# snap-research/InstantRestore

Measured on AMD Instinct MI355X. Metric: restored images/sec @512px, 4 refs, single-step; 1/2/4/8 MI355X, higher is better.
Workload: dtype bf16

## Files before the change

### instantrestore_amd/csrc/linear_tiled.hip

```cpp
#include <stdlib.h>
#include <type_traits>

#include "ir_common.h"
#include "ir_colstats.h"
#include "ir_kernels.h"

namespace {

constexpr int kTiledPitch = 144;

template <typename T, int WM, int WN, int MI, int NI, bool XF32, bool ILV, int KW = 1>
__global__ void __launch_bounds__(WM * WN * KW * 64, KW == 1 ? 2 : 1) linear_tiled_kernel(const LinearKParams p) {
  using Tr = ElemTraits<T>;
  using v8 = typename Tr::v8;
  using v4 = typename Tr::v4;
  constexpr int NW = WM * WN, NT = NW * 64;
  constexpr int BM = WM * MI * 32, BN = WN * NI * 32;
  constexpr int XT = BM * 128, WT = BN * 128, STAGE = XT + WT;
  constexpr int XP = BM / 8 / NW, WP = BN / 8 / NW;
  constexpr int XU = BM * 8 / NT;
  static_assert(BM % (8 * NW) == 0 && BN % (8 * NW) == 0, "pieces must divide over the waves");
  extern __shared__ __attribute__((aligned(16))) unsigned char dsm_tiled[];
  const int lane = threadIdx.x & 63;
  const int wid_all = __builtin_amdgcn_readfirstlane(threadIdx.x >> 6);
  const int kg = KW == 1 ? 0 : wid_all / NW;
  const int wid = KW == 1 ? wid_all : wid_all - kg * NW;
  const int tid = wid * 64 + lane;
  unsigned char* const smem = dsm_tiled + kg * (2 * STAGE);

  const int wm = wid / WN, wn = wid - wm * WN;
  const int hi = lane >> 5, lq = lane & 31;

  const int MT = (p.M + BM - 1) / BM, NTl = p.N / BN;
  const int logical = xcd_remap((int)blockIdx.x, MT * NTl);
  const int GM = p.nsplit;
  const int grp = logical / (GM * NTl), rem = logical - grp * (GM * NTl);
  const int gm = (MT - grp * GM) < GM ? (MT - grp * GM) : GM;
  const int tm = grp * GM + rem % gm, tn = rem / gm;
  const int m0 = tm * BM, n0 = tn * BN;
  const int rows_valid = (p.M - m0) < BM ? (p.M - m0) : BM;
  const int KT = (p.K >> 6) / KW;
  const int kt0 = kg * KT;

  const T* const wbase = (const T*)p.w + (int64_t)n0 * p.w_ld;
  const i32x4 wrs = make_rsrc_words(wbase, (unsigned)(((int64_t)(BN - 1) * p.w_ld + p.K) * 2));
  unsigned wvo[WP];
#pragma unroll
  for (int j = 0; j < WP; ++j) {
    const int row = 8 * (wid + j * NW) + (lane >> 3);
    wvo[j] = (unsigned)(row * p.w_ld * 2 + ((((lane & 7) ^ ((row >> 1) & 7))) << 4));
  }
  i32x4 xrs = wrs;
  unsigned xvo[XF32 ? 1 : XP];
  const float* xfp[XF32 ? XU : 1];
  int xlds[XF32 ? XU : 1];
  if constexpr (!XF32) {
    const T* const xbase = (const T*)p.x + (int64_t)m0 * p.x_ld;
    xrs = make_rsrc_words(xbase, (unsigned)(((int64_t)(rows_valid - 1) * p.x_ld + p.K) * 2));
#pragma unroll
    for (int j = 0; j < XP; ++j) {
      const int row = 8 * (wid + j * NW) + (lane >> 3);
      xvo[j] = (unsigned)(row * p.x_ld * 2 + ((((lane & 7) ^ ((row >> 1) & 7))) << 4));
    }
  } else {
#pragma unroll
    for (int j = 0; j < XU; ++j) {
      const int u = tid + j * NT, row = u >> 3, ch = u & 7;
      const int gr = (m0 + row) < p.M ? (m0 + row) : (p.M - 1);
      xfp[j] = (const float*)p.x + (int64_t)gr * p.x_ld + ch * 8;
      xlds[j] = row * 128 + ((ch ^ ((row >> 1) & 7)) << 4);
    }
  }
  constexpr int NPIECE = WP + (XF32 ? 0 : XP);
  auto issue_piece = [&](int j, int kt, int slot) {
    unsigned char* const sx = smem + slot * STAGE;
    if (j < WP) buffer_load_lds16_async(wrs, sx + XT + (wid + j * NW) * 1024, wvo[j] + (kt0 + kt) * 128);
    else if constexpr (!XF32) buffer_load_lds16_async(xrs, sx + (wid + (j - WP) * NW) * 1024, xvo[j - WP] + (kt0 + kt) * 128);
  };
  auto issue_dma = [&](int kt, int slot) {
#pragma unroll
    for (int j = 0; j < NPIECE; ++j) issue_piece(j, kt, slot);
  };
  f32x4 xr[XF32 ? XU : 1][2];
  auto load_x32 = [&](int kt) {
    if constexpr (XF32) {
#pragma unroll
      for (int j = 0; j < XU; ++j) {
        asm volatile("global_load_dwordx4 %0, %1, off" : "=v"(xr[j][0]) : "v"(xfp[j] + (kt0 + kt) * 64) : "memory");
        asm volatile("global_load_dwordx4 %0, %1, off offset:16" : "=v"(xr[j][1]) : "v"(xfp[j] + (kt0 + kt) * 64) : "memory");
      }
    }
  };
  auto put_x32 = [&](int slot) {
    if constexpr (XF32) {
      unsigned char* const sx = smem + slot * STAGE;
      asm volatile("s_waitcnt vmcnt(0)" : "+v"(xr[0][0]), "+v"(xr[0][1]) : : "memory");
#pragma unroll
      for (int j = 1; j < XU; ++j) asm volatile("" : "+v"(xr[j][0]), "+v"(xr[j][1]));
#pragma unroll
      for (int j = 0; j < XU; ++j) {
        const f32x8 f = __builtin_shufflevector(xr[j][0], xr[j][1], 0, 1, 2, 3, 4, 5, 6, 7);
        *(IR_LDS v8*)(IR_LDS unsigned char*)(sx + xlds[j]) = __builtin_convertvector(f, v8);
      }
    }
  };

  int fread[4];
#pragma unroll
  for (int ks = 0; ks < 4; ++ks) fread[ks] = lq * 128 + (((2 * ks + hi) ^ ((lq >> 1) & 7)) << 4);
  const int xrow0 = wm * (MI * 32) * 128, wrow0 = XT + wn * (NI * 32) * 128;

  f32x16 acc[MI][NI];
#pragma unroll
  for (int mi = 0; mi < MI; ++mi)
#pragma unroll
    for (int ni = 0; ni < NI; ++ni)
#pragma unroll
      for (int r = 0; r < 16; ++r) acc[mi][ni][r] = 0.f;

  constexpr int HALF_MFMA = 2 * MI * NI;
  constexpr int STRIDE = (HALF_MFMA / NPIECE) > 0 ? (HALF_MFMA / NPIECE) : 1;
  auto compute = [&](int slot, int dma_kt, int dma_slot) {
    const unsigned char* const st = smem + slot * STAGE;
    v8 wf[2][NI], xf[2][MI];
    auto rd = [&](int ks, int b) {
#pragma unroll
      for (int ni = 0; ni < NI; ++ni) wf[b][ni] = *(const IR_LDS v8*)(IR_LDS unsigned char*)(st + wrow0 + ni * 4096 + fread[ks]);
#pragma unroll
      for (int mi = 0; mi < MI; ++mi) xf[b][mi] = *(const IR_LDS v8*)(IR_LDS unsigned char*)(st + xrow0 + mi * 4096 + fread[ks]);
    };
    rd(0, 0);
#pragma unroll
    for (int ks = 0; ks < 4; ++ks) {
      if (ks + 1 < 4) rd(ks + 1, (ks + 1) & 1);
#pragma unroll
      for (int mi = 0; mi < MI; ++mi)
#pragma unroll
        for (int ni = 0; ni < NI; ++ni) {
          acc[mi][ni] = Tr::mfma(wf[ks & 1][ni], xf[ks & 1][mi], acc[mi][ni]);
          if constexpr (ILV) {
            const int m = ks * MI * NI + mi * NI + ni;
            if (m < HALF_MFMA && (m % STRIDE) == STRIDE - 1 && (m / STRIDE) < NPIECE) {
              __builtin_amdgcn_sched_barrier(0);
              if (dma_kt >= 0) issue_piece(m / STRIDE, dma_kt, dma_slot);
              __builtin_amdgcn_sched_barrier(0);
            }
            if (m == HALF_MFMA - 1) {
#pragma unroll
              for (int j = HALF_MFMA / STRIDE; j < NPIECE; ++j)
                if (dma_kt >= 0) issue_piece(j, dma_kt, dma_slot);
            }
          }
        }
    }
  };

  issue_dma(0, 0);
  load_x32(0);
  put_x32(0);
  asm volatile("s_waitcnt vmcnt(0)" ::: "memory");
  __syncthreads();
  for (int kt = 0; kt + 1 < KT; ++kt) {
    const int cur = kt & 1;
    if constexpr (!ILV) issue_dma(kt + 1, cur ^ 1);
    load_x32(kt + 1);
    compute(cur, kt + 1, cur ^ 1);
    put_x32(cur ^ 1);
    asm volatile("s_waitcnt vmcnt(0)" ::: "memory");
    __syncthreads();
  }
  compute((KT - 1) & 1, -1, 0);
  __syncthreads();
  if constexpr (KW == 2) {
    constexpr int HAND_OFF = 2 * STAGE;
    static_assert(2 * STAGE >= NW * MI * 32 * kTiledPitch, "epilogue staging must stay below the hand-over area");
    static_assert(2 * STAGE >= NW * MI * NI * 16 * 64 * 4, "hand-over area");
    unsigned char* const hand = dsm_tiled + HAND_OFF + wid * (MI * NI * 16 * 64 * 4) + lane * 16;
    if (kg == 1) {
#pragma unroll
      for (int mi = 0; mi < MI; ++mi)
#pragma unroll
        for (int ni = 0; ni < NI; ++ni)
#pragma unroll
          for (int g = 0; g < 4; ++g)
            *(f32x4_alias*)(hand + ((mi * NI + ni) * 4 + g) * 1024) = f32x4{acc[mi][ni][4 * g], acc[mi][ni][4 * g + 1], acc[mi][ni][4 * g + 2], acc[mi][ni][4 * g + 3]};
    }
    __syncthreads();
    if (kg == 1) return;
#pragma unroll
    for (int mi = 0; mi < MI; ++mi)
#pragma unroll
      for (int ni = 0; ni < NI; ++ni)
#pragma unroll
        for (int g = 0; g < 4; ++g) {
          const f32x4 o = *(const f32x4_alias*)(hand + ((mi * NI + ni) * 4 + g) * 1024);
#pragma unroll
          for (int i = 0; i < 4; ++i) acc[mi][ni][4 * g + i] += o[i];
        }
  }

  unsigned char* const tb = smem + wid * (MI * 32 * kTiledPitch);
  const int row_base = m0 + wm * (MI * 32);
  v4 bvs[NI][4];
  if (p.bias != nullptr) {
#pragma unroll
    for (int ni = 0; ni < NI; ++ni)
#pragma unroll
      for (int g = 0; g < 4; ++g) bvs[ni][g] = *(const v4*)((const T*)p.bias + n0 + wn * (NI * 32) + ni * 32 + 8 * g + 4 * hi);
  } else {
#pragma unroll
    for (int ni = 0; ni < NI; ++ni)
#pragma unroll
      for (int g = 0; g < 4; ++g) bvs[ni][g] = v4{0, 0, 0, 0};
  }
#pragma unroll
  for (int nh = 0; nh < NI / 2; ++nh) {
    const int ncol0 = n0 + wn * (NI * 32) + nh * 64;
#pragma unroll
    for (int n2 = 0; n2 < 2; ++n2) {
      const int ni = 2 * nh + n2;
      const float cs = (ncol0 + n2 * 32) < p.scale_cols ? p.col_scale : 1.0f;
#pragma unroll
      for (int g = 0; g < 4; ++g) {
        f32x4 bz;
#pragma unroll
        for (int i = 0; i < 4; ++i) bz[i] = (float)bvs[ni][g][i];
#pragma unroll
        for (int mi = 0; mi < MI; ++mi) {
          f32x4 f;
#pragma unroll
          for (int i = 0; i < 4; ++i) f[i] = acc[mi][ni][4 * g + i] * cs + bz[i];
          *(v4*)(tb + (mi * 32 + lq) * kTiledPitch + n2 * 64 + (8 * g + 4 * hi) * 2) = __builtin_convertvector(f, v4);
        }
      }
    }
    ir_wave_lds_fence();
    const int st_head = (ncol0 - p.st_col0) >> 6;
    const bool st_on = p.st_ws != nullptr && ncol0 >= p.st_col0 && st_head < (p.st_cols >> 6) && row_base < p.M;
    ColStatsAcc sacc;
#pragma unroll
    for (int j = 0; j < MI * 4; ++j) {
      const int r = 8 * j + (lane >> 3);
      const u32x4 v = *(const u32x4_alias*)(tb + r * kTiledPitch + (lane & 7) * 16);
      const int row = row_base + r;
      if (row < p.M) ir_store_y((u32x4*)((T*)p.y + (int64_t)row * p.y_ld + ncol0 + (lane & 7) * 8), v);
      if (st_on) {
        if (j == 0) ir_stats_first<T>(sacc, v);
        else ir_stats_add<T>(sacc, v);
      }
    }
    ir_wave_lds_fence();
    if (st_on) ir_stats_finish(sacc, p.st_ws + ((int64_t)(row_base / kStatsRows) * (p.st_cols >> 6) + st_head) * 128);
  }
}


template <typename T, bool XF32>
__global__ void __launch_bounds__(512, 2) linear_tiled_pp_kernel(const LinearKParams p) {
  using Tr = ElemTraits<T>;
  using v8 = typename Tr::v8;
  using v4 = typename Tr::v4;
  constexpr int NW = 8, NT = 512, WN = 2, MI = 2, NI = 4;
  constexpr int BM = 256, BN = 256;
  constexpr int XT = BM * 128, WT = BN * 128, STAGE = XT + WT;
  constexpr int XP = BM / 8 / NW, WP = BN / 8 / NW;
  constexpr int XU = BM * 8 / NT;
  constexpr int OUT_OFF = 2 * STAGE;
  extern __shared__ __attribute__((aligned(16))) unsigned char dsm_tiled_pp[];
  unsigned char* const smem = dsm_tiled_pp;

  const int tid = threadIdx.x;
  const int lane = tid & 63;
  const int wid = __builtin_amdgcn_readfirstlane(tid >> 6);
  const int grp = wid >> 2;
  const int wm = wid / WN, wn = wid - wm * WN;
  const int hi = lane >> 5, lq = lane & 31;
  const int KT = p.K >> 6;

  const int MT = (p.M + BM - 1) / BM, NTl = (p.N + BN - 1) / BN;
  const int ntiles = MT * NTl;
  const int xcd = blockIdx.x & 7, xs = blockIdx.x >> 3;
  const int q8 = ntiles >> 3, r8 = ntiles & 7;
  const int t_start = (xcd < r8) ? xcd * (q8 + 1) : r8 * (q8 + 1) + (xcd - r8) * q8;
  const int t_count = q8 + (xcd < r8 ? 1 : 0);
  const int wg_x = ((int)gridDim.x >> 3) + (xcd < ((int)gridDim.x & 7) ? 1 : 0);

  unsigned wvo[WP], xvo[XF32 ? 1 : XP];
  int xlds0 = 0;
#pragma unroll
  for (int j = 0; j < WP; ++j) {
    const int row = 8 * (wid + j * NW) + (lane >> 3);
    wvo[j] = (unsigned)(row * p.w_ld * 2 + ((((lane & 7) ^ ((row >> 1) & 7))) << 4));
  }
  if constexpr (!XF32) {
#pragma unroll
    for (int j = 0; j < XP; ++j) {
      const int row = 8 * (wid + j * NW) + (lane >> 3);
      xvo[j] = (unsigned)(row * p.x_ld * 2 + ((((lane & 7) ^ ((row >> 1) & 7))) << 4));
    }
  } else {
    const int row = tid >> 3, ch = tid & 7;
    xlds0 = row * 128 + ((ch ^ ((row >> 1) & 7)) << 4);
  }
  int fread[4];
#pragma unroll
  for (int ks = 0; ks < 4; ++ks) fread[ks] = lq * 128 + (((2 * ks + hi) ^ ((lq >> 1) & 7)) << 4);
  const int xrow0 = wm * (MI * 32) * 128, wrow0 = XT + wn * (NI * 32) * 128;

  int m0 = 0, n0 = 0;
  i32x4 wrs = {0, 0, 0, 0}, xrs = {0, 0, 0, 0};
  const float* xtile = nullptr;
  unsigned xoff[XF32 ? XU : 1];
  auto set_tile = [&](int logical) {
    const int GM = p.nsplit;
    const int tgrp = logical / (GM * NTl), rem = logical - tgrp * (GM * NTl);
    const int gm = (MT - tgrp * GM) < GM ? (MT - tgrp * GM) : GM;
    const int tm = tgrp * GM + rem % gm, tn = rem / gm;
    m0 = tm * BM; n0 = tn * BN;
    const int rows_valid = (p.M - m0) < BM ? (p.M - m0) : BM;
    const int cols_valid = (p.N - n0) < BN ? (p.N - n0) : BN;
    wrs = make_rsrc_words((const T*)p.w + (int64_t)n0 * p.w_ld, (unsigned)(((int64_t)(cols_valid - 1) * p.w_ld + p.K) * 2));
    if constexpr (!XF32) {
      xrs = make_rsrc_words((const T*)p.x + (int64_t)m0 * p.x_ld, (unsigned)(((int64_t)(rows_valid - 1) * p.x_ld + p.K) * 2));
    } else {
      xtile = (const float*)p.x + (int64_t)m0 * p.x_ld;
#pragma unroll
      for (int j = 0; j < XU; ++j) {
        const int row = (tid >> 3) + 64 * j;
        const int rr = row < rows_valid ? row : rows_valid - 1;
        xoff[j] = (unsigned)(rr * (int)p.x_ld + (tid & 7) * 8) * 4u;
      }
    }
  };
  f32x4 xr[XF32 ? XU : 1][2];
  auto issue_w = [&](int kt, int slot) {
    unsigned char* const sx = smem + slot * STAGE;
#pragma unroll
    for (int j = 0; j < WP; ++j) buffer_load_lds16_async(wrs, sx + XT + (wid + j * NW) * 1024, wvo[j] + kt * 128);
  };
  auto issue_x = [&](int kt, int slot) {
    if constexpr (!XF32) {
      unsigned char* const sx = smem + slot * STAGE;
#pragma unroll
      for (int j = 0; j < XP; ++j) buffer_load_lds16_async(xrs, sx + (wid + j * NW) * 1024, xvo[j] + kt * 128);
    } else {
#pragma unroll
      for (int j = 0; j < XU; ++j) {
        const unsigned o = xoff[j] + (unsigned)kt * 256u;
        asm volatile("s_nop 4\n\tglobal_load_dwordx4 %0, %1, %2" : "=v"(xr[j][0]) : "v"(o), "s"(xtile) : "memory");
        asm volatile("global_load_dwordx4 %0, %1, %2 offset:16" : "=v"(xr[j][1]) : "v"(o), "s"(xtile) : "memory");
      }
    }
  };
  auto land_stage = [&](int slot) {
    if constexpr (XF32) {
      unsigned char* const sx = smem + slot * STAGE;
      asm volatile("s_waitcnt vmcnt(0)" : "+v"(xr[0][0]), "+v"(xr[0][1]) : : "memory");
#pragma unroll
      for (int j = 1; j < XU; ++j) asm volatile("" : "+v"(xr[j][0]), "+v"(xr[j][1]));
#pragma unroll
      for (int j = 0; j < XU; ++j) {
        const f32x8 f = __builtin_shufflevector(xr[j][0], xr[j][1], 0, 1, 2, 3, 4, 5, 6, 7);
        *(IR_LDS v8*)(IR_LDS unsigned char*)(sx + xlds0 + j * 8192) = __builtin_convertvector(f, v8);
      }
    } else {
      asm volatile("s_waitcnt vmcnt(0)" ::: "memory");
    }
  };

  f32x16 acc[MI][NI];
  v8 wf[2][NI], xf[2][MI];
  auto load_frags = [&](int slot, int half) {
    const unsigned char* const st = smem + slot * STAGE;
#pragma unroll
    for (int q = 0; q < 2; ++q) {
#pragma unroll
      for (int ni = 0; ni < NI; ++ni) wf[q][ni] = *(const IR_LDS v8*)(IR_LDS unsigned char*)(st + wrow0 + ni * 4096 + fread[2 * half + q]);
#pragma unroll
      for (int mi = 0; mi < MI; ++mi) xf[q][mi] = *(const IR_LDS v8*)(IR_LDS unsigned char*)(st + xrow0 + mi * 4096 + fread[2 * half + q]);
    }
  };
  auto matrix_phase = [&]() {
    __builtin_amdgcn_s_setprio(1);
#pragma unroll
    for (int q = 0; q < 2; ++q)
#pragma unroll
      for (int mi = 0; mi < MI; ++mi)
#pragma unroll
        for (int ni = 0; ni < NI; ++ni) acc[mi][ni] = Tr::mfma(wf[q][ni], xf[q][mi], acc[mi][ni]);
    __builtin_amdgcn_s_setprio(0);
  };
  auto phase_end = [&]() {
    __builtin_amdgcn_sched_barrier(0);
    asm volatile("s_waitcnt lgkmcnt(0)" ::: "memory");
    __builtin_amdgcn_s_barrier();
    __builtin_amdgcn_sched_barrier(0);
  };
  auto epilogue = [&](int em0, int en0) {
    unsigned char* const tb = smem + OUT_OFF + wid * 4096;
#pragma unroll
    for (int nh = 0; nh < NI / 2; ++nh) {
      const int ncol0 = en0 + wn * (NI * 32) + nh * 64;
      if (ncol0 >= p.N) break;
      v4 bvs[2][4];
      if (p.bias != nullptr) {
#pragma unroll
        for (int n2 = 0; n2 < 2; ++n2)
#pragma unroll
          for (int g = 0; g < 4; ++g) bvs[n2][g] = *(const v4*)((const T*)p.bias + ncol0 + n2 * 32 + 8 * g + 4 * hi);
      } else {
#pragma unroll
        for (int n2 = 0; n2 < 2; ++n2)
#pragma unroll
          for (int g = 0; g < 4; ++g) bvs[n2][g] = v4{0, 0, 0, 0};
      }
      const int st_head = (ncol0 - p.st_col0) >> 6;
      const bool st_on = p.st_ws != nullptr && ncol0 >= p.st_col0 && st_head < (p.st_cols >> 6) && (em0 + wm * (MI * 32)) < p.M;
      ColStatsAcc sacc;
#pragma unroll
      for (int mi = 0; mi < MI; ++mi) {
#pragma unroll
        for (int half = 0; half < 2; ++half) {
          if ((lq >> 4) == half) {
#pragma unroll
            for (int n2 = 0; n2 < 2; ++n2) {
              const float cs = (ncol0 + n2 * 32) < p.scale_cols ? p.col_scale : 1.0f;
#pragma unroll
              for (int g = 0; g < 4; ++g) {
                f32x4 f;
#pragma unroll
                for (int i = 0; i < 4; ++i) f[i] = acc[mi][2 * nh + n2][4 * g + i] * cs + (float)bvs[n2][g][i];
                *(v4*)(tb + (lq & 15) * kTiledPitch + n2 * 64 + (8 * g + 4 * hi) * 2) = __builtin_convertvector(f, v4);
              }
            }
          }
          ir_wave_lds_fence();
#pragma unroll
          for (int j = 0; j < 2; ++j) {
            const int r = 8 * j + (lane >> 3);
            const u32x4 v = *(const u32x4_alias*)(tb + r * kTiledPitch + (lane & 7) * 16);
            const int row = em0 + wm * (MI * 32) + mi * 32 + half * 16 + r;
            if (row < p.M) ir_store_y((u32x4*)((T*)p.y + (int64_t)row * p.y_ld + ncol0 + (lane & 7) * 8), v);
            if (st_on) {
              if (mi == 0 && half == 0 && j == 0) ir_stats_first<T>(sacc, v);
              else ir_stats_add<T>(sacc, v);
            }
          }
          ir_wave_lds_fence();
        }
      }
      if (st_on) ir_stats_finish(sacc, p.st_ws + ((int64_t)((em0 + wm * (MI * 32)) / kStatsRows) * (p.st_cols >> 6) + st_head) * 128);
    }
  };

  if (xs >= t_count) return;
  set_tile(t_start + xs);
  issue_w(0, 0);
  issue_x(0, 0);
  for (int tl = xs; tl < t_count; tl += wg_x) {
#pragma unroll
    for (int mi = 0; mi < MI; ++mi)
#pragma unroll
      for (int ni = 0; ni < NI; ++ni)
#pragma unroll
        for (int r = 0; r < 16; ++r) acc[mi][ni][r] = 0.f;
    land_stage(0);
    asm volatile("s_waitcnt vmcnt(0)" ::: "memory");
    phase_end();
    load_frags(0, 0);
    if (KT > 1) { issue_w(1, 1); issue_x(1, 1); }
    if (grp == 1) phase_end();
    for (int kt = 0; kt < KT; ++kt) {
      const int cur = kt & 1;
      matrix_phase();
      phase_end();
      load_frags(cur, 1);
      if (kt + 1 < KT) land_stage(cur ^ 1);
      phase_end();
      matrix_phase();
      phase_end();
      if (kt + 1 < KT) {
        load_frags(cur ^ 1, 0);
        if (kt + 2 < KT) { issue_w(kt + 2, cur); issue_x(kt + 2, cur); }
      }
      phase_end();
    }
    if (grp == 0) phase_end();
    const int em0 = m0, en0 = n0;
    const bool more = tl + wg_x < t_count;
    if (more) {
      set_tile(t_start + tl + wg_x);
      issue_w(0, 0);
      if constexpr (!XF32) issue_x(0, 0);
    }
    epilogue(em0, en0);
    if constexpr (XF32) { if (more) issue_x(0, 0); }
  }
}


static int walk_group_rows() {
  static const int gm = [] { const char* e = getenv("IR_LIN_GM"); const int v = e ? atoi(e) : 0; return (v >= 1 && v <= 64) ? v : 4; }();
  return gm;
}

template <typename T, bool XF32>
hipError_t launch_pp(const LinearKParams& p0, hipStream_t s) {
  LinearKParams p = p0;
  p.nsplit = walk_group_rows();
  constexpr size_t dyn = 2 * (size_t)(256 + 256) * 128 + 8 * 4096;
  static IrOncePerDevice once;
  static std::atomic<int> n_cu[64];
  int dev = -1;
  const hipError_t ea = ir_opt_in_dynamic_lds(once, (const void*)linear_tiled_pp_kernel<T, XF32>, dyn, &dev);
  if (ea != hipSuccess) return ea;
  int cus = (dev >= 0 && dev < 64) ? n_cu[dev].load(std::memory_order_relaxed) : 0;
  if (cus <= 0) {
    if (hipDeviceGetAttribute(&cus, hipDeviceAttributeMultiprocessorCount, dev < 0 ? 0 : dev) != hipSuccess || cus <= 0) cus = 256;
    if (dev >= 0 && dev < 64) n_cu[dev].store(cus, std::memory_order_relaxed);
  }
  const int MT = (p.M + 255) / 256, NTl = (p.N + 255) / 256;
  const int ntiles = MT * NTl;
  static const bool persistent = [] { const char* e = getenv("IR_LIN_PERSISTENT"); return e == nullptr || e[0] != '0'; }();
  const int grid = (persistent && ntiles > cus) ? cus : ntiles;
  hipLaunchKernelGGL((linear_tiled_pp_kernel<T, XF32>), dim3((unsigned)grid), dim3(512), dyn, s, p);
  return hipGetLastError();
}

template <typename T, int WM, int WN, int MI, int NI, bool XF32, bool ILV, int KW = 1>
hipError_t launch_cfg(const LinearKParams& p0, hipStream_t s) {
  LinearKParams p = p0;
  p.nsplit = walk_group_rows();
  constexpr int BM = WM * MI * 32, BN = WN * NI * 32;
  constexpr size_t stage = (size_t)(BM + BN) * 128;
  constexpr size_t epi = (size_t)WM * WN * MI * 32 * kTiledPitch;
  constexpr size_t dyn = KW * 2 * stage > epi ? KW * 2 * stage : epi;
  if (KW == 2 && ((p.K >> 6) & 1)) return hipErrorInvalidValue;
  static IrOncePerDevice once;
  const hipError_t ea = ir_opt_in_dynamic_lds(once, (const void*)linear_tiled_kernel<T, WM, WN, MI, NI, XF32, ILV, KW>, dyn);
  if (ea != hipSuccess) return ea;
  const int MT = (p.M + BM - 1) / BM, NTl = p.N / BN;
  hipLaunchKernelGGL((linear_tiled_kernel<T, WM, WN, MI, NI, XF32, ILV, KW>), dim3((unsigned)(MT * NTl)), dim3(WM * WN * KW * 64), dyn, s, p);
  return hipGetLastError();
}

template <typename T, bool XF32>
hipError_t launch_x(const LinearKParams& p, int cfg, hipStream_t s) {
  constexpr bool I = true;
  switch (cfg) {
    case IR_LIN_TILE_256x128: return launch_cfg<T, 4, 2, 2, 2, XF32, I>(p, s);
    case IR_LIN_TILE_128x128: return launch_cfg<T, 2, 2, 2, 2, XF32, I>(p, s);
    case IR_LIN_TILE_128x64: return launch_cfg<T, 2, 1, 2, 2, XF32, I>(p, s);
    case IR_LIN_TILE_256x64: return launch_cfg<T, 4, 1, 2, 2, XF32, I>(p, s);
    case IR_LIN_TILE_64x128: return launch_cfg<T, 1, 2, 2, 2, XF32, I>(p, s);
    case IR_LIN_TILE_128x256: return launch_cfg<T, 2, 2, 2, 4, XF32, I>(p, s);
    case IR_LIN_TILE_128x128_K2: return launch_cfg<T, 2, 2, 2, 2, XF32, I, 2>(p, s);
    case IR_LIN_TILE_256x256: return launch_pp<T, XF32>(p, s);
    default: return hipErrorInvalidValue;
  }
}

}

int ir_linear_tiled_pick(int64_t M, int N, int K) {
  auto tiles = [&](int bm, int bn) { return ((M + bm - 1) / bm) * (int64_t)((N + bn - 1) / bn); };
  if (tiles(256, 256) >= 160) return IR_LIN_TILE_256x256;
  if (N % 128 == 0 && tiles(128, 128) >= 128 && tiles(128, 128) <= 256 && K >= 1024 && ((K >> 6) & 1) == 0) return IR_LIN_TILE_128x128_K2;
  if (N % 128 == 0) return tiles(128, 128) >= 128 ? IR_LIN_TILE_128x128 : IR_LIN_TILE_64x128;
  return tiles(256, 64) >= 512 ? IR_LIN_TILE_256x64 : IR_LIN_TILE_128x64;
}

bool ir_linear_tiled_cfg_ok(int cfg, int N) {
  switch (cfg) {
    case IR_LIN_TILE_256x128: case IR_LIN_TILE_128x128: case IR_LIN_TILE_64x128: case IR_LIN_TILE_128x128_K2: return N % 128 == 0;
    case IR_LIN_TILE_128x64: case IR_LIN_TILE_256x64: return N % 64 == 0;
    case IR_LIN_TILE_128x256: return N % 256 == 0;
    case IR_LIN_TILE_256x256: return N % 64 == 0;
    default: return false;
  }
}

hipError_t ir_launch_linear_tiled(const LinearKParams& p, int dtype, int cfg, hipStream_t s) {
  if (dtype == 1) return p.x_f32 ? launch_x<__bf16, true>(p, cfg, s) : launch_x<__bf16, false>(p, cfg, s);
  return p.x_f32 ? launch_x<_Float16, true>(p, cfg, s) : launch_x<_Float16, false>(p, cfg, s);
}
```

Measured before the change: 1223.

## Pipeline K-loads across persistent tiles and stream epilogue via buffer stores

Restructures the persistent GEMM loop into one continuous load pipeline over all (tile, k) steps. The next tile's first stages now overlap the current tile's epilogue instead of draining with vmcnt(0) at each tile boundary. The epilogue is rewritten to use buffer stores with a swizzled LDS staging layout, bias hoisted and specialised at compile time, and partial vmcnt waits that count the outstanding stores. Per-load offsets are recomputed from one base to cut VGPR use. This adds intricate counter bookkeeping, and a wrong vmcnt count would give races or stale data.

```diff
diff --git a/instantrestore_amd/csrc/linear_tiled.hip b/instantrestore_amd/csrc/linear_tiled.hip
--- a/instantrestore_amd/csrc/linear_tiled.hip
+++ b/instantrestore_amd/csrc/linear_tiled.hip
@@ -285,38 +285,35 @@
   const int t_count = q8 + (xcd < r8 ? 1 : 0);
   const int wg_x = ((int)gridDim.x >> 3) + (xcd < ((int)gridDim.x & 7) ? 1 : 0);
 
-  unsigned wvo[WP], xvo[XF32 ? 1 : XP];
+  unsigned wvo0, xvo0 = 0;
   int xlds0 = 0;
-#pragma unroll
-  for (int j = 0; j < WP; ++j) {
-    const int row = 8 * (wid + j * NW) + (lane >> 3);
-    wvo[j] = (unsigned)(row * p.w_ld * 2 + ((((lane & 7) ^ ((row >> 1) & 7))) << 4));
-  }
-  if constexpr (!XF32) {
-#pragma unroll
-    for (int j = 0; j < XP; ++j) {
-      const int row = 8 * (wid + j * NW) + (lane >> 3);
-      xvo[j] = (unsigned)(row * p.x_ld * 2 + ((((lane & 7) ^ ((row >> 1) & 7))) << 4));
-    }
-  } else {
+  {
+    const int row = 8 * wid + (lane >> 3);
+    const int swz = (((lane & 7) ^ ((row >> 1) & 7))) << 4;
+    wvo0 = (unsigned)(row * p.w_ld * 2 + swz);
+    if constexpr (!XF32) xvo0 = (unsigned)(row * p.x_ld * 2 + swz);
+  }
+  if constexpr (XF32) {
     const int row = tid >> 3, ch = tid & 7;
     xlds0 = row * 128 + ((ch ^ ((row >> 1) & 7)) << 4);
   }
-  int fread[4];
-#pragma unroll
-  for (int ks = 0; ks < 4; ++ks) fread[ks] = lq * 128 + (((2 * ks + hi) ^ ((lq >> 1) & 7)) << 4);
+  const int fread0 = lq * 128 + ((hi ^ ((lq >> 1) & 7)) << 4);
+  auto opaque = [](auto v) { asm volatile("" : "+v"(v)); return v; };
   const int xrow0 = wm * (MI * 32) * 128, wrow0 = XT + wn * (NI * 32) * 128;
 
-  int m0 = 0, n0 = 0;
+  auto tile_origin = [&](int logical, int& tm0, int& tn0) {
+    const int GM = p.nsplit;
+    const int tgrp = logical / (GM * NTl), rem = logical - tgrp * (GM * NTl);
+    const int gm = (MT - tgrp * GM) < GM ? (MT - tgrp * GM) : GM;
+    tm0 = (tgrp * GM + rem % gm) * BM;
+    tn0 = (rem / gm) * BN;
+  };
   i32x4 wrs = {0, 0, 0, 0}, xrs = {0, 0, 0, 0};
   const float* xtile = nullptr;
   unsigned xoff[XF32 ? XU : 1];
   auto set_tile = [&](int logical) {
-    const int GM = p.nsplit;
-    const int tgrp = logical / (GM * NTl), rem = logical - tgrp * (GM * NTl);
-    const int gm = (MT - tgrp * GM) < GM ? (MT - tgrp * GM) : GM;
-    const int tm = tgrp * GM + rem % gm, tn = rem / gm;
-    m0 = tm * BM; n0 = tn * BN;
+    int m0, n0;
+    tile_origin(logical, m0, n0);
     const int rows_valid = (p.M - m0) < BM ? (p.M - m0) : BM;
     const int cols_valid = (p.N - n0) < BN ? (p.N - n0) : BN;
     wrs = make_rsrc_words((const T*)p.w + (int64_t)n0 * p.w_ld, (unsigned)(((int64_t)(cols_valid - 1) * p.w_ld + p.K) * 2));
@@ -335,14 +332,16 @@
   f32x4 xr[XF32 ? XU : 1][2];
   auto issue_w = [&](int kt, int slot) {
     unsigned char* const sx = smem + slot * STAGE;
-#pragma unroll
-    for (int j = 0; j < WP; ++j) buffer_load_lds16_async(wrs, sx + XT + (wid + j * NW) * 1024, wvo[j] + kt * 128);
+    const unsigned o = opaque(wvo0);
+#pragma unroll
+    for (int j = 0; j < WP; ++j) buffer_load_lds16_async(wrs, sx + XT + (wid + j * NW) * 1024, o + (unsigned)(j * (8 * NW) * (int)p.w_ld * 2 + kt * 128));
   };
   auto issue_x = [&](int kt, int slot) {
     if constexpr (!XF32) {
       unsigned char* const sx = smem + slot * STAGE;
-#pragma unroll
-      for (int j = 0; j < XP; ++j) buffer_load_lds16_async(xrs, sx + (wid + j * NW) * 1024, xvo[j] + kt * 128);
+      const unsigned o = opaque(xvo0);
+#pragma unroll
+      for (int j = 0; j < XP; ++j) buffer_load_lds16_async(xrs, sx + (wid + j * NW) * 1024, o + (unsigned)(j * (8 * NW) * (int)p.x_ld * 2 + kt * 128));
     } else {
 #pragma unroll
       for (int j = 0; j < XU; ++j) {
@@ -352,10 +351,12 @@
       }
     }
   };
-  auto land_stage = [&](int slot) {
+  auto land_stage = [&](int slot, int younger) {
     if constexpr (XF32) {
       unsigned char* const sx = smem + slot * STAGE;
-      asm volatile("s_waitcnt vmcnt(0)" : "+v"(xr[0][0]), "+v"(xr[0][1]) : : "memory");
+      if (younger >= 16) asm volatile("s_waitcnt vmcnt(16)" : "+v"(xr[0][0]), "+v"(xr[0][1]) : : "memory");
+      else if (younger >= 8) asm volatile("s_waitcnt vmcnt(8)" : "+v"(xr[0][0]), "+v"(xr[0][1]) : : "memory");
+      else asm volatile("s_waitcnt vmcnt(0)" : "+v"(xr[0][0]), "+v"(xr[0][1]) : : "memory");
 #pragma unroll
       for (int j = 1; j < XU; ++j) asm volatile("" : "+v"(xr[j][0]), "+v"(xr[j][1]));
 #pragma unroll
@@ -364,20 +365,32 @@
         *(IR_LDS v8*)(IR_LDS unsigned char*)(sx + xlds0 + j * 8192) = __builtin_convertvector(f, v8);
       }
     } else {
-      asm volatile("s_waitcnt vmcnt(0)" ::: "memory");
+      if (younger >= 16) asm volatile("s_waitcnt vmcnt(16)" ::: "memory");
+      else if (younger >= 8) asm volatile("s_waitcnt vmcnt(8)" ::: "memory");
+      else asm volatile("s_waitcnt vmcnt(0)" ::: "memory");
     }
   };
 
   f32x16 acc[MI][NI];
   v8 wf[2][NI], xf[2][MI];
+  auto zero_acc = [&]() {
+#pragma unroll
+    for (int mi = 0; mi < MI; ++mi)
+#pragma unroll
+      for (int ni = 0; ni < NI; ++ni)
+#pragma unroll
+        for (int r = 0; r < 16; ++r) acc[mi][ni][r] = 0.f;
+  };
   auto load_frags = [&](int slot, int half) {
     const unsigned char* const st = smem + slot * STAGE;
+    const int f0 = opaque(fread0);
 #pragma unroll
     for (int q = 0; q < 2; ++q) {
-#pragma unroll
-      for (int ni = 0; ni < NI; ++ni) wf[q][ni] = *(const IR_LDS v8*)(IR_LDS unsigned char*)(st + wrow0 + ni * 4096 + fread[2 * half + q]);
-#pragma unroll
-      for (int mi = 0; mi < MI; ++mi) xf[q][mi] = *(const IR_LDS v8*)(IR_LDS unsigned char*)(st + xrow0 + mi * 4096 + fread[2 * half + q]);
+      const int fr = f0 ^ ((2 * half + q) << 5);
+#pragma unroll
+      for (int ni = 0; ni < NI; ++ni) wf[q][ni] = *(const IR_LDS v8*)(IR_LDS unsigned char*)(st + wrow0 + ni * 4096 + fr);
+#pragma unroll
+      for (int mi = 0; mi < MI; ++mi) xf[q][mi] = *(const IR_LDS v8*)(IR_LDS unsigned char*)(st + xrow0 + mi * 4096 + fr);
     }
   };
   auto matrix_phase = [&]() {
@@ -396,106 +409,154 @@
     __builtin_amdgcn_s_barrier();
     __builtin_amdgcn_sched_barrier(0);
   };
-  auto epilogue = [&](int em0, int en0) {
+  const unsigned y_8rows = (unsigned)(p.y_ld * 16);
+  auto epilogue_body = [&](int logical, auto bias_tag) -> int {
+    constexpr bool HAS_BIAS = decltype(bias_tag)::value;
+    int em0, en0;
+    tile_origin(logical, em0, en0);
+    const int rows_valid = (p.M - em0) < BM ? (p.M - em0) : BM;
+    const i32x4 yrs = make_rsrc_words((const T*)p.y + (int64_t)em0 * p.y_ld, (unsigned)((((int64_t)rows_valid - 1) * p.y_ld + p.N) * 2));
     unsigned char* const tb = smem + OUT_OFF + wid * 4096;
+    const int ln = opaque(lane), l31 = ln & 31, l8 = ln >> 3;
+    const int wb = l31 * 128 + ((l31 & 7) << 4) + (((ln >> 5) ^ ((l31 >> 3) & 1)) << 3);
+    const int rb = l8 * 128 + (((ln & 7) ^ l8) << 4);
+    const unsigned yl = (unsigned)((wm * (MI * 32) + l8) * (int)p.y_ld * 2 + (ln & 7) * 16);
+    int nstores = 0;
+    v4 bvs[NI / 2][2][4];
+    if constexpr (HAS_BIAS) {
+#pragma unroll
+      for (int nh = 0; nh < NI / 2; ++nh) {
+        const int c = en0 + wn * (NI * 32) + nh * 64;
+        const T* const bp = (const T*)p.bias + (c < p.N ? c : 0) + 4 * (ln >> 5);
+#pragma unroll
+        for (int n2 = 0; n2 < 2; ++n2)
+#pragma unroll
+          for (int g = 0; g < 4; ++g) bvs[nh][n2][g] = *(const v4*)(bp + n2 * 32 + 8 * g);
+      }
+#pragma unroll
+      for (int nh = 0; nh < NI / 2; ++nh)
+#pragma unroll
+        for (int n2 = 0; n2 < 2; ++n2)
+#pragma unroll
+          for (int g = 0; g < 4; ++g) asm volatile("" : "+v"(bvs[nh][n2][g]));
+    }
 #pragma unroll
     for (int nh = 0; nh < NI / 2; ++nh) {
       const int ncol0 = en0 + wn * (NI * 32) + nh * 64;
       if (ncol0 >= p.N) break;
-      v4 bvs[2][4];
-      if (p.bias != nullptr) {
-#pragma unroll
-        for (int n2 = 0; n2 < 2; ++n2)
-#pragma unroll
-          for (int g = 0; g < 4; ++g) bvs[n2][g] = *(const v4*)((const T*)p.bias + ncol0 + n2 * 32 + 8 * g + 4 * hi);
-      } else {
-#pragma unroll
-        for (int n2 = 0; n2 < 2; ++n2)
-#pragma unroll
-          for (int g = 0; g < 4; ++g) bvs[n2][g] = v4{0, 0, 0, 0};
-      }
       const int st_head = (ncol0 - p.st_col0) >> 6;
       const bool st_on = p.st_ws != nullptr && ncol0 >= p.st_col0 && st_head < (p.st_cols >> 6) && (em0 + wm * (MI * 32)) < p.M;
       ColStatsAcc sacc;
-#pragma unroll
-      for (int mi = 0; mi < MI; ++mi) {
-#pragma unroll
-        for (int half = 0; half < 2; ++half) {
-          if ((lq >> 4) == half) {
-#pragma unroll
-            for (int n2 = 0; n2 < 2; ++n2) {
-              const float cs = (ncol0 + n2 * 32) < p.scale_cols ? p.col_scale : 1.0f;
-#pragma unroll
-              for (int g = 0; g < 4; ++g) {
-                f32x4 f;
-#pragma unroll
-                for (int i = 0; i < 4; ++i) f[i] = acc[mi][2 * nh + n2][4 * g + i] * cs + (float)bvs[n2][g][i];
-                *(v4*)(tb + (lq & 15) * kTiledPitch + n2 * 64 + (8 * g + 4 * hi) * 2) = __builtin_convertvector(f, v4);
-              }
-            }
+      auto stage = [&](int mi) {
+#pragma unroll
+        for (int n2 = 0; n2 < 2; ++n2) {
+          const float cs = (ncol0 + n2 * 32) < p.scale_cols ? p.col_scale : 1.0f;
+#pragma unroll
+          for (int g = 0; g < 4; ++g) {
+            f32x4 f;
+#pragma unroll
+            for (int i = 0; i < 4; ++i) f[i] = acc[mi][2 * nh + n2][4 * g + i] * cs + (HAS_BIAS ? (float)bvs[nh][n2][g][i] : 0.f);
+            *(v4*)(tb + (wb ^ ((n2 * 4 + g) << 4))) = __builtin_convertvector(f, v4);
           }
-          ir_wave_lds_fence();
-#pragma unroll
-          for (int j = 0; j < 2; ++j) {
-            const int r = 8 * j + (lane >> 3);
-            const u32x4 v = *(const u32x4_alias*)(tb + r * kTiledPitch + (lane & 7) * 16);
-            const int row = em0 + wm * (MI * 32) + mi * 32 + half * 16 + r;
-            if (row < p.M) ir_store_y((u32x4*)((T*)p.y + (int64_t)row * p.y_ld + ncol0 + (lane & 7) * 8), v);
-            if (st_on) {
-              if (mi == 0 && half == 0 && j == 0) ir_stats_first<T>(sacc, v);
-              else ir_stats_add<T>(sacc, v);
-            }
+        }
+      };
+      auto fetch = [&](u32x4 (&v)[4]) {
+#pragma unroll
+        for (int j = 0; j < 4; ++j) {
+          const u32x4 t = *(const u32x4_alias*)(tb + rb + j * 1024);
+          v[j] = (j & 1) ? u32x4{t[2], t[3], t[0], t[1]} : t;
+        }
+      };
+      auto send = [&](int mi, const u32x4 (&v)[4]) {
+#pragma unroll
+        for (int j = 0; j < 4; ++j) buffer_store16_async(yrs, v[j], yl + (unsigned)(mi * 4 + j) * y_8rows, (unsigned)ncol0 * 2u);
+        if (st_on) {
+#pragma unroll
+          for (int j = 0; j < 4; ++j) {
+            if (mi == 0 && j == 0) ir_stats_first<T>(sacc, v[j]);
+            else ir_stats_add<T>(sacc, v[j]);
           }
-          ir_wave_lds_fence();
         }
-      }
+      };
+      u32x4 v[4];
+      stage(0);
+      ir_wave_lds_fence();
+      fetch(v);
+      ir_wave_lds_fence();
+      stage(1);
+      ir_wave_lds_fence();
+      send(0, v);
+      fetch(v);
+      ir_wave_lds_fence();
+      send(1, v);
+      nstores += 8;
       if (st_on) ir_stats_finish(sacc, p.st_ws + ((int64_t)((em0 + wm * (MI * 32)) / kStatsRows) * (p.st_cols >> 6) + st_head) * 128);
     }
+    return nstores;
+  };
+  auto epilogue = [&](int logical) -> int {
+    return p.bias != nullptr ? epilogue_body(logical, std::true_type{}) : epilogue_body(logical, std::false_type{});
   };
 
   if (xs >= t_count) return;
+  const int steps = ((t_count - xs + wg_x - 1) / wg_x) * KT;
+  int is = 0, ikt = 0, itl = xs;
   set_tile(t_start + xs);
-  issue_w(0, 0);
-  issue_x(0, 0);
+  auto issue_next_w = [&]() {
+    if (is < steps) issue_w(ikt, is & 1);
+  };
+  auto issue_next_x = [&]() {
+    if (is < steps) {
+      issue_x(ikt, is & 1);
+      ++is;
+      if (++ikt == KT) {
+        ikt = 0;
+        itl += wg_x;
+        if (itl < t_count) set_tile(t_start + itl);
+      }
+    } else if constexpr (XF32) {
+#pragma unroll
+      for (int j = 0; j < XU; ++j) asm volatile("" : "=v"(xr[j][0]), "=v"(xr[j][1]));
+    }
+  };
+  auto issue_next = [&]() { issue_next_w(); issue_next_x(); };
+  zero_acc();
+  issue_next();
+  land_stage(0, 0);
+  phase_end();
+  load_frags(0, 0);
+  issue_next();
+  if (grp == 1) phase_end();
+  int gs = 0, younger = 0;
   for (int tl = xs; tl < t_count; tl += wg_x) {
-#pragma unroll
-    for (int mi = 0; mi < MI; ++mi)
-#pragma unroll
-      for (int ni = 0; ni < NI; ++ni)
-#pragma unroll
-        for (int r = 0; r < 16; ++r) acc[mi][ni][r] = 0.f;
-    land_stage(0);
-    asm volatile("s_waitcnt vmcnt(0)" ::: "memory");
-    phase_end();
-    load_frags(0, 0);
-    if (KT > 1) { issue_w(1, 1); issue_x(1, 1); }
-    if (grp == 1) phase_end();
-    for (int kt = 0; kt < KT; ++kt) {
-      const int cur = kt & 1;
+    for (int kt = 0; kt < KT; ++kt, ++gs) {
+      const int cur = gs & 1;
+      const bool has_next = gs + 1 < steps;
       matrix_phase();
       phase_end();
       load_frags(cur, 1);
-      if (kt + 1 < KT) land_stage(cur ^ 1);
+      if (has_next) land_stage(cur ^ 1, younger);
+      younger = 0;
       phase_end();
       matrix_phase();
       phase_end();
       if (kt + 1 < KT) {
         load_frags(cur ^ 1, 0);
-        if (kt + 2 < KT) { issue_w(kt + 2, cur); issue_x(kt + 2, cur); }
-      }
-      phase_end();
-    }
-    if (grp == 0) phase_end();
-    const int em0 = m0, en0 = n0;
-    const bool more = tl + wg_x < t_count;
-    if (more) {
-      set_tile(t_start + tl + wg_x);
-      issue_w(0, 0);
-      if constexpr (!XF32) issue_x(0, 0);
-    }
-    epilogue(em0, en0);
-    if constexpr (XF32) { if (more) issue_x(0, 0); }
-  }
+        issue_next();
+        phase_end();
+      } else {
+        issue_next_w();
+        if constexpr (!XF32) issue_next_x();
+        if (grp == 0) phase_end();
+        younger = epilogue(t_start + tl);
+        if constexpr (XF32) { issue_next_x(); younger = 0; }
+        zero_acc();
+        load_frags(cur ^ 1, 0);
+        if (grp == 1) phase_end();
+      }
+    }
+  }
+  if (grp == 0) phase_end();
 }
 
 
```

After: 1223, median of 2. No clear change (-0.0%).
